# DoHoonKim8/stark-verifier

Hardware: AMD Instinct MI355X
Metric: recursive plonky2 proofs/sec (Semaphore d=20) (higher is better)
Workload: dtype u64 (Goldilocks field, integer); 1 GPU; recursive: per unit one Semaphore signal (group 2^20, n=2^13, blowup 8, 28 FRI queries, 16 PoW bits, zk) + the recursive proof verifying it (n=2^14, same FRI parameters); 128 units per GPU per step, 10 prover contexts per GPU; all_gather of (nullifier|topic) + Poseidon aggregation root per step; parallelism=independent proofs sharded over ranks, no data-path collective, exchange=none (one rank): gl355_aggregation_root over the local leaves, units_proven_in_process=1674

## Files before the change

stark-verifier_amd/csrc/merkle.hip:

```cpp
#include "gl355_internal.h"
#include "poseidon.cuh"
#include "merkle_common.cuh"

namespace gl355 {


__global__ void __launch_bounds__(256) poseidon_permute_kernel(uint64_t* states, uint64_t count) {
    const uint64_t i = blockIdx.x * (uint64_t)blockDim.x + threadIdx.x;
    if (i >= count) return;
    uint64_t s[12];
#pragma unroll
    for (int k = 0; k < 12; k++) s[k] = states[i * 12 + k];
    psd_permute(s);
#pragma unroll
    for (int k = 0; k < 12; k++) states[i * 12 + k] = gl_canon(s[k]);
}


#ifndef PSD_LEAF_WAVES
#define PSD_LEAF_WAVES 4
#endif
__global__ void __launch_bounds__(256) __attribute__((amdgpu_waves_per_eu(PSD_LEAF_WAVES))) hash_leaves_kernel(LeafArgs a) {
    const uint64_t i = blockIdx.x * (uint64_t)blockDim.x + threadIdx.x;
    if (i >= a.n_leaves) return;
    uint64_t s[12];
#pragma unroll
    for (int k = 0; k < 12; k++) s[k] = 0;
    const uint32_t len = a.leaf_len;
    uint64_t d[4];
    if (len <= 4 && !a.always_hash) {
        for (uint32_t k = 0; k < 4; k++) {
            uint64_t v = 0;
            if (k < len) v = leaf_elem(a, i, k);
            d[k] = gl_canon(v);
        }
    } else {
        for (uint32_t off = 0; off < len; off += 8) {
            const uint32_t m = min(8u, len - off);
#pragma unroll
            for (uint32_t k = 0; k < 8; k++) {
                if (k < m) s[k] = leaf_elem(a, i, off + k);
            }
            psd_permute(s);
        }
#pragma unroll
        for (int k = 0; k < 4; k++) d[k] = gl_canon(s[k]);
    }
    uint64_t* dst;
    if (a.linear) dst = a.out + i * 4;
    else if (a.sub_bits == 0) dst = a.cap + i * 4;
    else {
        const uint64_t sub_leaves = 1ull << a.sub_bits;
        const uint64_t t = i >> a.sub_bits, k = i & (sub_leaves - 1);
        dst = a.out + (t * 2 * (sub_leaves - 1) + digest_slot(0, k)) * 4;
    }
    *reinterpret_cast<ulonglong2*>(dst) = make_ulonglong2(d[0], d[1]);
    *reinterpret_cast<ulonglong2*>(dst + 2) = make_ulonglong2(d[2], d[3]);
}

__global__ void __launch_bounds__(256) merkle_level_kernel(uint64_t* digests, uint64_t* cap, uint32_t sub_bits,
                                                          uint32_t layer, uint64_t n_nodes ) {
    const uint64_t g = blockIdx.x * (uint64_t)blockDim.x + threadIdx.x;
    if (g >= n_nodes) return;
    const uint64_t sub_leaves = 1ull << sub_bits;
    const uint64_t per = sub_leaves >> layer;
    const uint64_t t = g / per, k = g % per;
    uint64_t* tree = digests + t * 2 * (sub_leaves - 1) * 4;
    const uint64_t child = digest_slot(layer - 1, 2 * k);
    const ulonglong2 l0 = *reinterpret_cast<const ulonglong2*>(tree + child * 4);
    const ulonglong2 l1 = *reinterpret_cast<const ulonglong2*>(tree + child * 4 + 2);
    const ulonglong2 r0 = *reinterpret_cast<const ulonglong2*>(tree + child * 4 + 4);
    const ulonglong2 r1 = *reinterpret_cast<const ulonglong2*>(tree + child * 4 + 6);
    uint64_t s[12] = {l0.x, l0.y, l1.x, l1.y, r0.x, r0.y, r1.x, r1.y, 0, 0, 0, 0};
    psd_permute(s);
    uint64_t* dst = (layer == sub_bits) ? cap + t * 4 : tree + digest_slot(layer, k) * 4;
    *reinterpret_cast<ulonglong2*>(dst) = make_ulonglong2(gl_canon(s[0]), gl_canon(s[1]));
    *reinterpret_cast<ulonglong2*>(dst + 2) = make_ulonglong2(gl_canon(s[2]), gl_canon(s[3]));
}

__device__ __constant__ const uint32_t PSD_CIRC_DEV[12] = {17, 15, 41, 16, 2, 28, 13, 13, 39, 18, 34, 20};

#define GL_WAVE_LDS_SYNC()                                      \
    do {                                                        \
        __builtin_amdgcn_fence(__ATOMIC_SEQ_CST, "wavefront");  \
        __builtin_amdgcn_wave_barrier();                        \
    } while (0)
#ifndef PSD_LANES_FORM
#define PSD_LANES_FORM -1
#endif
template <int FORM>
GL_DEV uint64_t psd_permute_lanes(uint64_t s, int li, uint64_t* ring ) {
    const bool active = li < 12;
    const int me = active ? li : 0;
    s = gl_add_canonical(s, PSD_ALL_RC[me]);
    auto dense_round = [&](int r, bool full) {
        const uint64_t rc_next = PSD_ALL_RC[12 * (r + 1) + me];
        if (full || li == 0) s = psd_sbox(s);
        if (active) { ring[me] = s; ring[me + 12] = s; }
        GL_WAVE_LDS_SYNC();
        uint64_t al = (uint32_t)rc_next, ah = rc_next >> 32;
#pragma unroll
        for (int j = 0; j < 12; j++) {
            const uint64_t x = ring[me + j];
            const uint32_t c = PSD_CIRC_DEV[j] + ((me == 0 && j == 0) ? 8u : 0u);
            al += (uint64_t)(uint32_t)x * c;
            ah += (uint64_t)(uint32_t)(x >> 32) * c;
        }
        GL_WAVE_LDS_SYNC();
        s = psd_recombine(al, ah);
    };
#if !defined(__HIP_DEVICE_COMPILE__) || GL_MUL_VARIANT != 1
#pragma unroll 1
    for (int r = 0; r < 30; r++) dense_round(r, r < 4 || r >= 26);
#else
    if constexpr (FORM == 0) {
#pragma unroll 1
        for (int r = 0; r < 30; r++) dense_round(r, r < 4 || r >= 26);
        return s;
    }
    const uint32_t c_elem0 = PSD_CIRC_DEV[(12 - me) % 12] + (me == 0 ? 8u : 0u);
#pragma unroll 1
    for (int r = 0; r < 4; r++) dense_round(r, true);
#pragma unroll 1
    for (int r = 4; r < 26; r++) {
        const uint64_t rc_next = PSD_ALL_RC[12 * (r + 1) + me];
        if (active) { const uint64_t pub = li == 0 ? 0 : s; ring[me] = pub; ring[me + 12] = pub; }
        GL_WAVE_LDS_SYNC();
        uint64_t xr[12];
#pragma unroll
        for (int j = 0; j < 12; j++) xr[j] = ring[me + j];
        uint64_t al = (uint32_t)rc_next, ah = rc_next >> 32;
        auto term = [&](int j) {
            al += (uint64_t)(uint32_t)xr[j] * PSD_CIRC_DEV[j];
            ah += (uint64_t)(uint32_t)(xr[j] >> 32) * PSD_CIRC_DEV[j];
        };
        const uint64_t x2 = gl_mul_fill(s, s, [&](int k) { term(k); });
        uint64_t p34[2];
        { const uint64_t pa[2] = {s, x2}, pb[2] = {x2, x2}; gl_mul2_fill(pa, pb, p34, [&](int k) { term(5 + k); }); }
        const uint64_t x7 = gl_mul_fill(p34[0], p34[1], [&](int k) { if (k < 2) term(10 + k); else asm volatile("s_nop 1"); });
        const uint32_t x0l = __builtin_amdgcn_update_dpp(0u, (uint32_t)x7, 0x150, 0xf, 0xf, false);
        const uint32_t x0h = __builtin_amdgcn_update_dpp(0u, (uint32_t)(x7 >> 32), 0x150, 0xf, 0xf, false);
        al += (uint64_t)x0l * c_elem0;
        ah += (uint64_t)x0h * c_elem0;
        GL_WAVE_LDS_SYNC();
        s = psd_recombine(al, ah);
    }
#pragma unroll 1
    for (int r = 26; r < 30; r++) dense_round(r, true);
#endif
    return s;
}

template <int FORM>
__global__ void __launch_bounds__(64) merkle_level_lanes_kernel(uint64_t* digests, uint64_t* cap, uint32_t sub_bits,
                                                               uint32_t layer, uint64_t n_nodes) {
    __shared__ uint64_t rings[4][24];
    const int li = threadIdx.x & 15, grp = threadIdx.x >> 4;
    uint64_t g = blockIdx.x * 4ull + grp;
    const bool valid = g < n_nodes;
    if (!valid) g = 0;
    const uint64_t sub_leaves = 1ull << sub_bits;
    const uint64_t per = sub_leaves >> layer;
    const uint64_t t = g / per, k = g % per;
    uint64_t* tree = digests + t * 2 * (sub_leaves - 1) * 4;
    const uint64_t child = digest_slot(layer - 1, 2 * k);
    uint64_t s = (li < 8) ? tree[child * 4 + li] : 0;
    s = psd_permute_lanes<FORM>(s, li, rings[grp]);
    if (valid && li < 4) {
        uint64_t* dst = (layer == sub_bits) ? cap + t * 4 : tree + digest_slot(layer, k) * 4;
        dst[li] = gl_canon(s);
    }
}

#define MERKLE_TOP_LEVELS 8
template <int FORM>
__global__ void __launch_bounds__(1024) merkle_top_kernel(uint64_t* digests, uint64_t* cap, uint32_t sub_bits, uint32_t layer0, uint32_t n_levels) {
    __shared__ uint64_t rings[64][24];
    __shared__ uint64_t lvl[2][(1 << (MERKLE_TOP_LEVELS - 1)) * 4];
    const int li = threadIdx.x & 15, grp = threadIdx.x >> 4;
    const int wave_first_grp = (threadIdx.x >> 6) << 2;
    const uint64_t sub_leaves = 1ull << sub_bits;
    const uint64_t t = blockIdx.x;
    uint64_t* tree = digests + t * 2 * (sub_leaves - 1) * 4;
    int cur = 0;
    for (uint32_t l = 0; l < n_levels; l++) {
        const uint32_t layer = layer0 + l;
        const int cnt = 1 << (n_levels - 1 - l);
        for (int base = 0; base < cnt; base += 64) {
            if (base + wave_first_grp < cnt) {
                const bool valid = base + grp < cnt;
                const int j = valid ? base + grp : 0;
                uint64_t s = 0;
                if (li < 8) s = (l == 0) ? tree[digest_slot(layer - 1, 2 * (uint64_t)j) * 4 + li] : lvl[cur][(2 * j) * 4 + li];
                s = psd_permute_lanes<FORM>(s, li, rings[grp]);
                if (valid && li < 4) {
                    const uint64_t v = gl_canon(s);
                    lvl[cur ^ 1][j * 4 + li] = v;
                    uint64_t* dst = (layer == sub_bits) ? cap + t * 4 : tree + digest_slot(layer, (uint64_t)j) * 4;
                    dst[li] = v;
                }
            }
        }
        __syncthreads();
        cur ^= 1;
    }
}

__global__ void __launch_bounds__(256) two_to_one_kernel(const uint64_t* l, const uint64_t* r, uint64_t n, uint64_t* out) {
    const uint64_t i = blockIdx.x * (uint64_t)blockDim.x + threadIdx.x;
    if (i >= n) return;
    uint64_t s[12] = {l[4 * i], l[4 * i + 1], l[4 * i + 2], l[4 * i + 3],
                      r[4 * i], r[4 * i + 1], r[4 * i + 2], r[4 * i + 3], 0, 0, 0, 0};
    psd_permute(s);
#pragma unroll
    for (int k = 0; k < 4; k++) out[4 * i + k] = gl_canon(s[k]);
}

__global__ void __launch_bounds__(256) pow_grind_kernel(const uint64_t* state, uint32_t pos, uint32_t bits,
                                                       uint64_t start, unsigned long long* best) {
    const uint64_t w = start + blockIdx.x * (uint64_t)blockDim.x + threadIdx.x;
    if (w > __hip_atomic_load(best, __ATOMIC_RELAXED, __HIP_MEMORY_SCOPE_AGENT)) return;
    uint64_t s[12];
#pragma unroll
    for (int k = 0; k < 12; k++) s[k] = state[k];
#pragma unroll
    for (int k = 0; k < 12; k++) if ((uint32_t)k == pos) s[k] = w;
    psd_permute(s);
    const uint64_t resp = gl_canon(s[7]);
    if (bits == 0 || (resp >> (64 - bits)) == 0) atomicMin(best, (unsigned long long)w);
}

__global__ void open_batch_kernel(const uint64_t* lde, uint64_t stride, uint32_t leaf_len, const uint64_t* digests,
                                  uint32_t log_n, uint32_t cap_height, const uint64_t* idx, uint32_t idx_shift,
                                  uint64_t* leaves_out, uint64_t leaf_out_stride, uint64_t* sib_out, uint64_t sib_out_stride) {
    const uint64_t index = idx[blockIdx.x] >> idx_shift;
    const uint32_t layers = log_n - cap_height;
    for (uint32_t c = threadIdx.x; c < leaf_len; c += blockDim.x)
        leaves_out[(uint64_t)blockIdx.x * leaf_out_stride + c] = stride ? lde[(uint64_t)c * stride + index] : lde[index * leaf_len + c];
    const uint64_t sub_leaves = 1ull << layers;
    const uint64_t* tree = digests + (index >> layers) * 2 * (sub_leaves - 1) * 4;
    const uint64_t k0 = index & (sub_leaves - 1);
    for (uint32_t e = threadIdx.x; e < layers * 4; e += blockDim.x) {
        const uint32_t layer = e >> 2;
        const uint64_t k = (k0 >> layer) ^ 1;
        sib_out[(uint64_t)blockIdx.x * sib_out_stride + layer * 4 + (e & 3)] = tree[digest_slot(layer, k) * 4 + (e & 3)];
    }
}

int32_t open_batch_dev(Ctx* ctx, const uint64_t* lde, uint64_t stride, uint32_t leaf_len, const uint64_t* digests,
                       uint32_t log_n, uint32_t cap_height, const uint64_t* idx_dev, uint32_t n_idx, uint64_t* leaves_out,
                       uint64_t* sib_out) {
    if (n_idx == 0) return GL355_OK;
    ProfScope ps(ctx, "open_batch", (uint64_t)n_idx * (leaf_len * 16 + (log_n - cap_height) * 64));
    hipLaunchKernelGGL(open_batch_kernel, dim3(n_idx), dim3(64), 0, ctx->stream, lde, stride, leaf_len, digests, log_n,
                       cap_height, idx_dev, 0u, leaves_out, (uint64_t)leaf_len, sib_out, (uint64_t)(log_n - cap_height) * 4);
    GL355_HIP(ctx, hipGetLastError());
    return GL355_OK;
}
int32_t open_batch_ex_dev(Ctx* ctx, const uint64_t* leaves, uint64_t stride, uint32_t leaf_len, const uint64_t* digests,
                          uint32_t log_n, uint32_t cap_height, const uint64_t* idx_dev, uint32_t idx_shift, uint32_t n_idx,
                          uint64_t* leaves_out, uint64_t leaf_out_stride, uint64_t* sib_out, uint64_t sib_out_stride) {
    if (n_idx == 0) return GL355_OK;
    ProfScope ps(ctx, "open_batch", (uint64_t)n_idx * (leaf_len * 16 + (log_n - cap_height) * 64));
    hipLaunchKernelGGL(open_batch_kernel, dim3(n_idx), dim3(64), 0, ctx->stream, leaves, stride, leaf_len, digests, log_n,
                       cap_height, idx_dev, idx_shift, leaves_out, leaf_out_stride, sib_out, sib_out_stride);
    GL355_HIP(ctx, hipGetLastError());
    return GL355_OK;
}

int32_t poseidon_permute_dev(Ctx* ctx, uint64_t* states, uint64_t count) {
    if (count == 0) return GL355_OK;
    hipLaunchKernelGGL(poseidon_permute_kernel, dim3((uint32_t)((count + 255) / 256)), dim3(256), 0, ctx->stream, states, count);
    GL355_HIP(ctx, hipGetLastError());
    return GL355_OK;
}

static int32_t launch_leaves(Ctx* ctx, const LeafArgs& a) {
    if (a.n_leaves == 0) return GL355_OK;
    hipLaunchKernelGGL(hash_leaves_kernel, dim3((uint32_t)((a.n_leaves + 255) / 256)), dim3(256), 0, ctx->stream, a);
    GL355_HIP(ctx, hipGetLastError());
    return GL355_OK;
}

int32_t hash_leaves_dev(Ctx* ctx, const uint64_t* leaves, uint64_t n_leaves, uint32_t leaf_len, bool col_major,
                        uint64_t col_stride, uint64_t* digests) {
    LeafArgs a;
    memset(&a, 0, sizeof a);
    a.leaves = leaves; a.n_leaves = n_leaves; a.leaf_len = leaf_len; a.col_major = col_major;
    a.stride = col_major ? col_stride : leaf_len;
    a.out = digests; a.linear = 1;
    return launch_leaves(ctx, a);
}

int32_t hash_no_pad_dev(Ctx* ctx, const uint64_t* inputs, uint64_t n, uint32_t len, uint64_t* digests) {
    LeafArgs a;
    memset(&a, 0, sizeof a);
    a.leaves = inputs; a.n_leaves = n; a.leaf_len = len; a.col_major = 0; a.stride = len;
    a.out = digests; a.linear = 1; a.always_hash = 1;
    return launch_leaves(ctx, a);
}

int32_t two_to_one_dev(Ctx* ctx, const uint64_t* l, const uint64_t* r, uint64_t n, uint64_t* out) {
    if (n == 0) return GL355_OK;
    hipLaunchKernelGGL(two_to_one_kernel, dim3((uint32_t)((n + 255) / 256)), dim3(256), 0, ctx->stream, l, r, n, out);
    GL355_HIP(ctx, hipGetLastError());
    return GL355_OK;
}

int32_t merkle_build_dev(Ctx* ctx, const uint64_t* leaves, uint64_t n_leaves, uint32_t leaf_len, bool col_major,
                         uint64_t col_stride, uint32_t cap_height, uint64_t* digests, uint64_t* cap) {
// ... 77 lines not shown
```

stark-verifier_amd/csrc/poseidon.cuh:

```cuda
#pragma once
#include "gl_field.cuh"

#define PSD_TABLE_QUAL __device__ __constant__ const
#include "poseidon_tables.h"

namespace gl355 {

#ifndef PSD_SBOX_INTERLEAVE
#define PSD_SBOX_INTERLEAVE 1
#endif
#ifndef PSD_SBOX_WIDTH
#define PSD_SBOX_WIDTH 4
#endif
GL_DEV uint64_t psd_sbox(uint64_t x) {
#if PSD_SBOX_INTERLEAVE && defined(__HIP_DEVICE_COMPILE__) && GL_MUL_VARIANT == 1
    const uint64_t x2 = gl_sqr(x);
    const uint64_t a[2] = {x, x2}, b[2] = {x2, x2};
    uint64_t r[2];
    gl_mul_multi<2>(a, b, r);
    return gl_mul(r[0], r[1]);
#else
    uint64_t x2 = gl_sqr(x), x4 = gl_sqr(x2), x3 = gl_mul(x, x2);
    return gl_mul(x3, x4);
#endif
}
GL_DEV void psd_sbox2(uint64_t& x, uint64_t& y) {
#if PSD_SBOX_INTERLEAVE && defined(__HIP_DEVICE_COMPILE__) && GL_MUL_VARIANT == 1
    uint64_t sq[2];
    { const uint64_t a[2] = {x, y}; gl_mul_multi<2>(a, a, sq); }
    uint64_t r[4];
    { const uint64_t a[4] = {x, sq[0], y, sq[1]}, b[4] = {sq[0], sq[0], sq[1], sq[1]}; gl_mul_multi<4>(a, b, r); }
    { const uint64_t a[2] = {r[0], r[2]}, b[2] = {r[1], r[3]}; uint64_t o[2]; gl_mul_multi<2>(a, b, o); x = o[0]; y = o[1]; }
#else
    x = psd_sbox(x); y = psd_sbox(y);
#endif
}

GL_DEV uint64_t psd_recombine(uint64_t al, uint64_t ah) {
#if GL_MUL_VARIANT == 1 && defined(__HIP_DEVICE_COMPILE__)
    uint32_t t1 = (uint32_t)(al >> 32), top;
    asm("v_add_co_u32_e32 %0, vcc, %0, %2\n\t" GL_HAZARD_NOP "v_addc_co_u32_e32 %1, vcc, 0, %3, vcc"
        : "+v"(t1), "=v"(top) : "v"((uint32_t)ah), "v"((uint32_t)(ah >> 32)) : "vcc");
    return gl_dev_add_mul_eps(((uint64_t)t1 << 32) | (uint32_t)al, top);
#else
    const uint64_t mid = ah << 32;
    const uint32_t top = (uint32_t)(ah >> 32);
    const uint64_t r0 = al + mid;
    const uint64_t carry = r0 < mid ? 1u : 0u;
    const uint64_t t = (uint64_t)(top + carry) * GL_EPS;
    uint64_t r1 = r0 + t;
    if (r1 < t) r1 += GL_EPS;
    return r1;
#endif
}

GL_DEV void psd_sbox4(uint64_t& x0, uint64_t& x1, uint64_t& x2, uint64_t& x3) {
#if PSD_SBOX_INTERLEAVE && defined(__HIP_DEVICE_COMPILE__) && GL_MUL_VARIANT == 1
    const uint64_t a[4] = {x0, x1, x2, x3};
    uint64_t sq[4], c3[4], c4[4], o[4];
    gl_mul_multi<4>(a, a, sq);
    gl_mul_multi<4>(a, sq, c3);
    gl_mul_multi<4>(sq, sq, c4);
    gl_mul_multi<4>(c3, c4, o);
    x0 = o[0]; x1 = o[1]; x2 = o[2]; x3 = o[3];
#else
    x0 = psd_sbox(x0); x1 = psd_sbox(x1); x2 = psd_sbox(x2); x3 = psd_sbox(x3);
#endif
}
template <int N>
GL_DEV void psd_recombine_multi(const uint64_t (&al)[N], const uint64_t (&ah)[N], uint64_t (&out)[N]) {
#if GL_MUL_VARIANT == 1 && defined(__HIP_DEVICE_COMPILE__)
    static_assert(N >= 3, "three or more: no wait states of their own");
    uint32_t t1[N], top[N], m[N];
    uint64_t c[N], r[N];
#pragma unroll
    for (int j = 0; j < N; j++) {
        asm("v_add_co_u32_e64 %0, %1, %2, %3" : "=v"(t1[j]), "=s"(c[j]) : "v"((uint32_t)(al[j] >> 32)), "v"((uint32_t)ah[j]));
        __builtin_amdgcn_sched_barrier(0);
    }
#pragma unroll
    for (int j = 0; j < N; j++) {
        asm("v_addc_co_u32_e64 %0, %1, 0, %2, %1" : "=v"(top[j]), "+s"(c[j]) : "v"((uint32_t)(ah[j] >> 32)));
        __builtin_amdgcn_sched_barrier(0);
    }
#pragma unroll
    for (int j = 0; j < N; j++) {
        const uint64_t x = ((uint64_t)t1[j] << 32) | (uint32_t)al[j];
        asm("v_mad_u64_u32 %0, %1, %2, -1, %3" : "=v"(r[j]), "=s"(c[j]) : "v"(top[j]), "v"(x));
        __builtin_amdgcn_sched_barrier(0);
    }
#pragma unroll
    for (int j = 0; j < N; j++) {
        asm("v_cndmask_b32_e64 %0, 0, -1, %1" : "=v"(m[j]) : "s"(c[j]));
        __builtin_amdgcn_sched_barrier(0);
    }
#pragma unroll
    for (int j = 0; j < N; j++) out[j] = r[j] + (uint64_t)m[j];
#else
#pragma unroll
    for (int j = 0; j < N; j++) out[j] = psd_recombine(al[j], ah[j]);
#endif
}

#define PSD_MDS_CHAIN(C0)                                                                                  \
    "v_mad_u64_u32 %0, %1, %2, " #C0 ", %14\n\tv_mad_u64_u32 %0, %1, %3, 15, %0\n\tv_mad_u64_u32 %0, %1, %4, 41, %0\n\t" \
    "v_mad_u64_u32 %0, %1, %5, 16, %0\n\tv_mad_u64_u32 %0, %1, %6, 2, %0\n\tv_mad_u64_u32 %0, %1, %7, 28, %0\n\t"      \
    "v_mad_u64_u32 %0, %1, %8, 13, %0\n\tv_mad_u64_u32 %0, %1, %9, 13, %0\n\tv_mad_u64_u32 %0, %1, %10, 39, %0\n\t"    \
    "v_mad_u64_u32 %0, %1, %11, 18, %0\n\tv_mad_u64_u32 %0, %1, %12, 34, %0\n\tv_mad_u64_u32 %0, %1, %13, 20, %0"
template <int R>
GL_DEV uint64_t psd_mds_chain(const uint32_t (&x)[12], uint64_t addend) {
    uint64_t acc, unused;
#define PSD_X(i) "v"(x[((i) + R) % 12])
    if constexpr (R == 0)
        asm(PSD_MDS_CHAIN(25) : "=&v"(acc), "=&s"(unused) : PSD_X(0), PSD_X(1), PSD_X(2), PSD_X(3), PSD_X(4), PSD_X(5), PSD_X(6),
            PSD_X(7), PSD_X(8), PSD_X(9), PSD_X(10), PSD_X(11), "s"(addend));
    else
        asm(PSD_MDS_CHAIN(17) : "=&v"(acc), "=&s"(unused) : PSD_X(0), PSD_X(1), PSD_X(2), PSD_X(3), PSD_X(4), PSD_X(5), PSD_X(6),
            PSD_X(7), PSD_X(8), PSD_X(9), PSD_X(10), PSD_X(11), "s"(addend));
#undef PSD_X
    return acc;
}
template <int R>
GL_DEV void psd_mds_rows(uint64_t (&s)[12], const uint32_t (&lo)[12], const uint32_t (&hi)[12], const uint64_t* rc) {
    if constexpr (R < 12) {
#if PSD_SBOX_INTERLEAVE
        const uint64_t c0 = rc[R], c1 = rc[R + 1], c2 = rc[R + 2], c3 = rc[R + 3];
        const uint64_t al[4] = {psd_mds_chain<R>(lo, (uint32_t)c0), psd_mds_chain<R + 1>(lo, (uint32_t)c1), psd_mds_chain<R + 2>(lo, (uint32_t)c2),
                                psd_mds_chain<R + 3>(lo, (uint32_t)c3)};
        const uint64_t ah[4] = {psd_mds_chain<R>(hi, c0 >> 32), psd_mds_chain<R + 1>(hi, c1 >> 32), psd_mds_chain<R + 2>(hi, c2 >> 32),
                                psd_mds_chain<R + 3>(hi, c3 >> 32)};
        uint64_t o[4];
        __builtin_amdgcn_sched_barrier(0);
        psd_recombine_multi<4>(al, ah, o);
        s[R] = o[0]; s[R + 1] = o[1]; s[R + 2] = o[2]; s[R + 3] = o[3];
        psd_mds_rows<R + 4>(s, lo, hi, rc);
#else
        const uint64_t c = rc[R];
        s[R] = psd_recombine(psd_mds_chain<R>(lo, (uint32_t)c), psd_mds_chain<R>(hi, c >> 32));
        psd_mds_rows<R + 1>(s, lo, hi, rc);
#endif
    }
}
GL_DEV void psd_mds(uint64_t (&s)[12], const uint64_t* rc) {
    uint32_t lo[12], hi[12];
#pragma unroll
    for (int i = 0; i < 12; i++) { lo[i] = (uint32_t)s[i]; hi[i] = (uint32_t)(s[i] >> 32); }
    psd_mds_rows<0>(s, lo, hi, rc);
}


#undef PSD_TABLE_QUAL
#define PSD_TABLE_QUAL __device__ __constant__
#include "poseidon_ktables.h"

GL_DEV void psd_split(uint64_t x, uint32_t (&l)[3]) {
    const uint32_t lo = (uint32_t)x, hi = (uint32_t)(x >> 32);
    l[0] = lo & 0x3FFFFFu;
    l[1] = __builtin_amdgcn_alignbit(hi, lo, 22) & 0x3FFFFFu;
    l[2] = hi >> 12;
}
typedef const __attribute__((address_space(4))) uint64_t* psd_ktab;
GL_DEV void psd_mac(uint64_t& lo, uint64_t& hi, const uint32_t (&l)[3], const uint64_t (&c)[3]) {
    const uint64_t c0 = c[0], c1 = c[1], c2 = c[2];
#if defined(__HIP_DEVICE_COMPILE__)
    uint64_t unused;
    asm("v_mad_u64_u32 %0, %2, %3, %9, %0\n\tv_mad_u64_u32 %1, %2, %4, %9, %1\n\t"
        "v_mad_u64_u32 %0, %2, %5, %10, %0\n\tv_mad_u64_u32 %1, %2, %6, %10, %1\n\t"
        "v_mad_u64_u32 %0, %2, %7, %11, %0\n\tv_mad_u64_u32 %1, %2, %8, %11, %1"
        : "+v"(lo), "+v"(hi), "=&s"(unused)
        : "s"((uint32_t)c0), "s"((uint32_t)(c0 >> 32)), "s"((uint32_t)c1), "s"((uint32_t)(c1 >> 32)), "s"((uint32_t)c2), "s"((uint32_t)(c2 >> 32)),
          "v"(l[0]), "v"(l[1]), "v"(l[2]));
#else
    lo += (uint64_t)l[0] * (uint32_t)c0 + (uint64_t)l[1] * (uint32_t)c1 + (uint64_t)l[2] * (uint32_t)c2;
    hi += (uint64_t)l[0] * (uint32_t)(c0 >> 32) + (uint64_t)l[1] * (uint32_t)(c1 >> 32) + (uint64_t)l[2] * (uint32_t)(c2 >> 32);
#endif
}
GL_DEV void psd_mac_first(uint64_t& lo, uint64_t& hi, const uint32_t (&l)[3], const uint64_t (&c)[3], const uint64_t (&add)[2]) {
    const uint64_t c0 = c[0], c1 = c[1], c2 = c[2];
#if defined(__HIP_DEVICE_COMPILE__)
    uint64_t unused;
    asm("v_mov_b64 %0, %12\n\tv_mov_b64 %1, %13\n\t"
        "v_mad_u64_u32 %0, %2, %3, %9, %0\n\tv_mad_u64_u32 %1, %2, %4, %9, %1\n\t"
        "v_mad_u64_u32 %0, %2, %5, %10, %0\n\tv_mad_u64_u32 %1, %2, %6, %10, %1\n\t"
        "v_mad_u64_u32 %0, %2, %7, %11, %0\n\tv_mad_u64_u32 %1, %2, %8, %11, %1"
        : "=&v"(lo), "=&v"(hi), "=&s"(unused)
        : "s"((uint32_t)c0), "s"((uint32_t)(c0 >> 32)), "s"((uint32_t)c1), "s"((uint32_t)(c1 >> 32)), "s"((uint32_t)c2), "s"((uint32_t)(c2 >> 32)),
          "v"(l[0]), "v"(l[1]), "v"(l[2]), "s"(add[0]), "s"(add[1]));
#else
    lo = add[0]; hi = add[1];
    psd_mac(lo, hi, l, c);
#endif
}
#ifndef PSD_K_GROUP
#define PSD_K_GROUP 5
#endif
struct PsdK {
    uint64_t w[PSD_K_GROUP][3];
    uint64_t a[2];
};
template <int N, bool WITH_ADD>
GL_DEV void psd_kload(PsdK& k, psd_ktab c, psd_ktab add) {
#pragma unroll
    for (int i = 0; i < N; i++)
#pragma unroll
        for (int j = 0; j < 3; j++) k.w[i][j] = c[3 * i + j];
    if constexpr (WITH_ADD) { k.a[0] = add[0]; k.a[1] = add[1]; }
}
template <int NX, bool HAS_NEXT, int XCAP>
GL_DEV void psd_dot(const uint32_t (&ul)[11][3], const uint32_t (&xl)[XCAP][3], psd_ktab c, PsdK& k, psd_ktab add_next, uint64_t& lo, uint64_t& hi) {
    constexpr int G = PSD_K_GROUP, NT = 11 + NX, NG = (NT + G - 1) / G;
    PsdK cur = k;
#pragma unroll
    for (int g = 0; g < NG; g++) {
        const int n = NT - g * G < G ? NT - g * G : G;
        PsdK nxt;
#pragma unroll
        for (int i = 0; i < G; i++) {
            const int t = g * G + i;
            if (t == 0) psd_mac_first(lo, hi, ul[0], cur.w[0], cur.a);
            else if (i < n) {
                if (t < 11) psd_mac(lo, hi, ul[t], cur.w[i]);
                else psd_mac(lo, hi, xl[t - 11], cur.w[i]);
            }
            if (i == 0) {
                __builtin_amdgcn_sched_barrier(0);
                if (g + 1 < NG) {
                    if (NT - (g + 1) * G >= G) psd_kload<G, false>(nxt, c + 3 * (g + 1) * G, add_next);
                    else psd_kload<(NT % G ? NT % G : G), false>(nxt, c + 3 * (g + 1) * G, add_next);
                } else if constexpr (HAS_NEXT) {
                    psd_kload<G, true>(nxt, c + 3 * NT, add_next);
                }
                __builtin_amdgcn_sched_barrier(0);
            }
        }
        __builtin_amdgcn_sched_barrier(0);
        if (g + 1 < NG || HAS_NEXT) cur = nxt;
    }
    if constexpr (HAS_NEXT) k = cur;
}
template <int J>
GL_DEV void psd_block_lane0(const uint32_t (&ul)[11][3], uint32_t (&xl)[PSD_K_BLOCK][3], psd_ktab mac, psd_ktab add, PsdK& k) {
    if constexpr (J < PSD_K_BLOCK) {
        uint64_t lo, hi;
        psd_dot<J, true>(ul, xl, mac + 3 * (11 * (J - 1) + (J - 1) * J / 2), k, add + 2 * J, lo, hi);
        psd_split(psd_sbox(psd_recombine(lo, hi)), xl[J]);
        __builtin_amdgcn_sched_barrier(0);
        psd_block_lane0<J + 1>(ul, xl, mac, add, k);
    }
}
template <int R>
GL_DEV void psd_block_out(uint64_t (&s)[12], const uint32_t (&ul)[11][3], const uint32_t (&xl)[PSD_K_BLOCK][3], psd_ktab mac, psd_ktab add, PsdK& k) {
    constexpr int B = PSD_K_BLOCK;
    if constexpr (R < 12) {
        uint64_t lo, hi;
        psd_dot<B, (R < 11)>(ul, xl, mac + 3 * (11 * (B - 1) + (B - 1) * B / 2 + (11 + B) * R), k, add + 2 * (B + R), lo, hi);
        s[R] = psd_recombine(lo, hi);
        __builtin_amdgcn_sched_barrier(0);
        psd_block_out<R + 1>(s, ul, xl, mac, add, k);
    }
}
GL_DEV void psd_partial_rounds_block(uint64_t (&s)[12]) {
    constexpr int B = PSD_K_BLOCK;
#pragma unroll 1
    for (int blk = 0; blk < 22 / B; blk++) {
        psd_ktab add = (psd_ktab)PSD_K_ADD + blk * 2 * (B - 1 + 12);
        psd_ktab mac = (psd_ktab)PSD_K_MAC;
        asm volatile("" : "+s"(mac));
        PsdK k;
        psd_kload<PSD_K_GROUP, true>(k, mac, add);
        __builtin_amdgcn_sched_barrier(0);
        uint32_t ul[11][3], xl[B][3];
#pragma unroll
        for (int i = 0; i < 11; i++) psd_split(s[i + 1], ul[i]);
        psd_split(psd_sbox(s[0]), xl[0]);
        __builtin_amdgcn_sched_barrier(0);
        psd_block_lane0<1>(ul, xl, mac, add, k);
        psd_block_out<0>(s, ul, xl, mac, add, k);
    }
}

#ifndef PSD_PARTIAL_FORM
#define PSD_PARTIAL_FORM 1
#endif
#ifndef PSD_ROUNDS_PER_ITER
#define PSD_ROUNDS_PER_ITER 2
#endif
template <bool FULL>
GL_DEV void psd_dense_rounds(uint64_t (&s)[12], int r0, int r1) {
#pragma unroll 1
    for (int r = r0; r < r1; r += PSD_ROUNDS_PER_ITER) {
#pragma unroll
        for (int h = 0; h < PSD_ROUNDS_PER_ITER; h++) {
            if (FULL) {
#pragma unroll
#if PSD_SBOX_WIDTH == 4
                for (int i = 0; i < 12; i += 4) psd_sbox4(s[i], s[i + 1], s[i + 2], s[i + 3]);
#else
                for (int i = 0; i < 12; i += 2) psd_sbox2(s[i], s[i + 1]);
#endif
            } else {
                s[0] = psd_sbox(s[0]);
            }
            psd_mds(s, &PSD_ALL_RC[12 * (r + h + 1)]);
        }
    }
}
GL_DEV void psd_permute(uint64_t (&s)[12]) {
#pragma unroll
    for (int i = 0; i < 12; i++) s[i] = gl_add_canonical(s[i], PSD_ALL_RC[i]);
    psd_dense_rounds<true>(s, 0, 4);
#if PSD_PARTIAL_FORM == 1
    psd_partial_rounds_block(s);
#else
    psd_dense_rounds<false>(s, 4, 26);
#endif
    psd_dense_rounds<true>(s, 26, 30);
}

struct PsdSponge {
    uint64_t s[12];
    GL_DEV void init() {
#pragma unroll
        for (int i = 0; i < 12; i++) s[i] = 0;
    }
};

}
```

stark-verifier_amd/csrc/prover_batch.hip:

```cpp
#include "gl355_internal.h"
#include "blinding.cuh"
#include "poseidon.cuh"

using namespace gl355;

namespace gl355 {

constexpr uint32_t MAXB = GL355_MAX_UNITS;

struct BOracle {
    Ctx* ctx = nullptr;
    uint32_t B = 0, log_n = 0, rate_bits = 0, batch = 0, leaf_len = 0, cap_height = 0;
    uint64_t* base = nullptr;
    uint64_t *coeffs = nullptr, *lde = nullptr, *salt = nullptr, *digests = nullptr, *cap = nullptr;
    uint64_t n_dig = 0;
    ~BOracle() { if (base && ctx) ctx->release(base); }
    int32_t alloc(Ctx* c, uint32_t b, uint32_t lg, uint32_t rb, uint32_t bat, bool salted, uint32_t cap_h) {
        ctx = c; B = b; log_n = lg; rate_bits = rb; batch = bat; leaf_len = bat + (salted ? GL355_SALT_SIZE : 0); cap_height = cap_h;
        const uint64_t n = 1ull << lg, N = n << rb, n_cap = 1ull << cap_h;
        n_dig = 2 * (N - n_cap);
        const uint64_t total = (uint64_t)B * ((uint64_t)bat * n + (uint64_t)leaf_len * N + n_dig * 4 + n_cap * 4);
        void* p = nullptr;
        GL355_TRY(c->alloc(total * 8, &p));
        base = reinterpret_cast<uint64_t*>(p);
// ... 254 lines not shown
        if (other < DEEP_BLK) add = gl2_mul(gl2_make(sh[2 * other], sh[2 * other + 1]), gl2_make(z_pow2[2 * s], z_pow2[2 * s + 1]));
        __syncthreads();
        c = gl2_add(c, add);
        sh[2 * tid] = c.c0; sh[2 * tid + 1] = c.c1;
        __syncthreads();
    }
    uint64_t* v = a.v + (uint64_t)u * a.n * 2;
    if (k < a.n) { v[2 * k] = c.c0; v[2 * k + 1] = c.c1; }
    if (tid == 0) { uint64_t* t = a.totals + ((uint64_t)u * a.n_blocks + blockIdx.x) * 2; t[0] = c.c0; t[1] = c.c1; }
}
__global__ void deep_carry_units_kernel(DeepArgs a) {
    const uint32_t u = blockIdx.x;
    if (threadIdx.x != 0) return;
    const uint64_t* tab = deep_tab_u(a, u);
    const uint64_t* z_pows = tab + 2 * ((uint64_t)(a.n_alpha + 1) + (uint64_t)a.point * (8 + DEEP_BLK + 1) + 8);
    const gl2 zb = gl2_make(z_pows[2 * DEEP_BLK], z_pows[2 * DEEP_BLK + 1]);
    const uint64_t* totals = a.totals + (uint64_t)u * a.n_blocks * 2;
    uint64_t* carry = a.carry + (uint64_t)u * a.n_blocks * 2;
    gl2 c = gl2_make(0, 0);
    for (uint64_t blk = a.n_blocks; blk-- > 0;) {
        carry[2 * blk] = c.c0; carry[2 * blk + 1] = c.c1;
        c = gl2_add(gl2_make(totals[2 * blk], totals[2 * blk + 1]), gl2_mul(zb, c));
    }
}
__global__ void __launch_bounds__(DEEP_BLK) deep_finish_units_kernel(DeepArgs a) {
    const uint64_t k = blockIdx.x * (uint64_t)DEEP_BLK + threadIdx.x;
    if (k >= a.n) return;
    const uint32_t u = blockIdx.y;
    const uint64_t* tab = deep_tab_u(a, u);
    const uint64_t* z_pows = tab + 2 * ((uint64_t)(a.n_alpha + 1) + (uint64_t)a.point * (8 + DEEP_BLK + 1) + 8);
    const uint64_t* v = a.v + (uint64_t)u * a.n * 2;
    const uint64_t* carry = a.carry + (uint64_t)u * a.n_blocks * 2;
    gl2 q = gl2_make(0, 0);
    const uint64_t j = k + 1;
    if (j < a.n) {
        const uint64_t blk = j / DEEP_BLK, off = j % DEEP_BLK;
        const gl2 cr = gl2_make(carry[2 * blk], carry[2 * blk + 1]);
        const uint64_t e = DEEP_BLK - off;
        q = gl2_add(gl2_make(v[2 * j], v[2 * j + 1]), gl2_mul(gl2_make(z_pows[2 * e], z_pows[2 * e + 1]), cr));
    }
    uint64_t* acc0 = a.acc + (uint64_t)u * 2 * a.n;
    uint64_t* acc1 = acc0 + a.n;
    const gl2 shift = gl2_make(tab[2 * a.n_polys], tab[2 * a.n_polys + 1]);
    const gl2 r = gl2_canon(gl2_add(gl2_mul(gl2_make(acc0[k], acc1[k]), shift), q));
    acc0[k] = r.c0; acc1[k] = r.c1;
}

__global__ void fri_leaves_units_kernel(const uint64_t* cols , uint64_t len, uint64_t* leaves ) {
    const uint64_t i = blockIdx.x * (uint64_t)blockDim.x + threadIdx.x;
    if (i >= len / 2) return;
    const uint32_t u = blockIdx.y;
    const uint64_t* c0 = cols + (uint64_t)u * 2 * len;
    const uint64_t* c1 = c0 + len;
    const ulonglong2 a = *reinterpret_cast<const ulonglong2*>(c0 + 2 * i);
    const ulonglong2 b = *reinterpret_cast<const ulonglong2*>(c1 + 2 * i);
    uint64_t* dst = leaves + ((uint64_t)u * (len / 2) + i) * 4;
    *reinterpret_cast<ulonglong2*>(dst) = make_ulonglong2(a.x, b.x);
    *reinterpret_cast<ulonglong2*>(dst + 2) = make_ulonglong2(a.y, b.y);
}
__global__ void fri_fold_units_kernel(const uint64_t* cols , uint64_t len, UnitVals beta, uint64_t* out ) {
    const uint64_t k = blockIdx.x * (uint64_t)blockDim.x + threadIdx.x;
    const uint64_t half = len / 2;
    if (k >= half) return;
    const uint32_t u = blockIdx.y;
    const uint64_t* c0 = cols + (uint64_t)u * 2 * len;
    const uint64_t* c1 = c0 + len;
    const ulonglong2 a = *reinterpret_cast<const ulonglong2*>(c0 + 2 * k);
    const ulonglong2 b = *reinterpret_cast<const ulonglong2*>(c1 + 2 * k);
    const gl2 r = gl2_canon(gl2_add(gl2_make(a.x, b.x), gl2_mul(gl2_make(a.y, b.y), gl2_make(beta.v[u * 4], beta.v[u * 4 + 1]))));
    uint64_t* o0 = out + (uint64_t)u * 2 * half;
    o0[k] = r.c0; o0[half + k] = r.c1;
}
struct PowArgs { uint64_t state[MAXB * 12]; uint32_t pos[MAXB]; uint32_t todo[MAXB]; uint32_t bits; uint64_t start; unsigned long long* best; };
__global__ void __launch_bounds__(256) pow_grind_units_kernel(PowArgs a) {
    const uint32_t u = blockIdx.y;
    if (!a.todo[u]) return;
    const uint64_t w = a.start + blockIdx.x * (uint64_t)blockDim.x + threadIdx.x;
    if (w > __hip_atomic_load(a.best + u, __ATOMIC_RELAXED, __HIP_MEMORY_SCOPE_AGENT)) return;
    uint64_t s[12];
#pragma unroll
    for (int k = 0; k < 12; k++) s[k] = a.state[u * 12 + k];
#pragma unroll
    for (int k = 0; k < 12; k++) if ((uint32_t)k == a.pos[u]) s[k] = w;
    psd_permute(s);
    const uint64_t resp = gl_canon(s[7]);
    if (a.bits == 0 || (resp >> (64 - a.bits)) == 0) atomicMin(a.best + u, (unsigned long long)w);
}

struct OpenArgs { OView o; uint64_t N; uint32_t lde_bits, cap_height, n_idx; const uint64_t* idx ; uint64_t* leaves; uint64_t* sibs; };
__global__ void open_units_kernel(OpenArgs a) {
    const uint32_t q = blockIdx.x, u = blockIdx.y;
    const uint64_t index = a.idx[(uint64_t)u * a.n_idx + q];
    const uint32_t layers = a.lde_bits - a.cap_height;
    const uint64_t* lde = a.o.lde + (uint64_t)u * a.o.lde_us;
    const uint64_t* salt = a.o.salt ? a.o.salt + (uint64_t)u * a.o.salt_us : nullptr;
    uint64_t* lo = a.leaves + ((uint64_t)u * a.n_idx + q) * a.o.leaf_len;
    for (uint32_t c = threadIdx.x; c < a.o.leaf_len; c += blockDim.x)
        lo[c] = c < a.o.batch ? lde[(uint64_t)c * a.N + index] : salt[(uint64_t)(c - a.o.batch) * a.N + index];
    const uint64_t sub_leaves = 1ull << layers;
    const uint64_t* tree = a.o.digests + (uint64_t)u * a.o.dig_us + (index >> layers) * 2 * (sub_leaves - 1) * 4;
    const uint64_t k0 = index & (sub_leaves - 1);
    uint64_t* so = a.sibs + ((uint64_t)u * a.n_idx + q) * layers * 4;
    for (uint32_t e = threadIdx.x; e < layers * 4; e += blockDim.x) {
        const uint32_t layer = e >> 2;
        const uint64_t k = (k0 >> layer) ^ 1;
        so[e] = tree[digest_slot(layer, k) * 4 + (e & 3)];
    }
}
struct OpenFriArgs {
    const uint64_t* trees; uint64_t leaf_off[32], dig_off[32];
    uint64_t sib_off[32], sib_total;
    uint32_t lde_bits, cap_height, n_idx, n_layers;
    const uint64_t* idx; uint64_t* evals ; uint64_t* sibs ;
};
__global__ void open_fri_units_kernel(OpenFriArgs a) {
    const uint32_t q = blockIdx.x, u = blockIdx.y, l = blockIdx.z;
    const uint64_t index = a.idx[(uint64_t)u * a.n_idx + q] >> (l + 1);
    const uint32_t log_nl = a.lde_bits - 1 - l, layers = log_nl - a.cap_height;
    const uint64_t nl = 1ull << log_nl, n_cap = 1ull << a.cap_height;
    const uint64_t* leaves = a.trees + a.leaf_off[l] + (uint64_t)u * nl * 4;
    const uint64_t* digs = a.trees + a.dig_off[l] + (uint64_t)u * 2 * (nl - n_cap) * 4;
    uint64_t* ev = a.evals + (((uint64_t)u * a.n_idx + q) * a.n_layers + l) * 4;
    if (threadIdx.x < 4) ev[threadIdx.x] = leaves[index * 4 + threadIdx.x];
    const uint64_t sub_leaves = 1ull << layers;
    const uint64_t* tree = digs + (index >> layers) * 2 * (sub_leaves - 1) * 4;
    const uint64_t k0 = index & (sub_leaves - 1);
    uint64_t* so = a.sibs + ((uint64_t)u * a.n_idx + q) * a.sib_total + a.sib_off[l];
    for (uint32_t e = threadIdx.x; e < layers * 4; e += blockDim.x) {
        const uint32_t layer = e >> 2;
        const uint64_t k = (k0 >> layer) ^ 1;
        so[e] = tree[digest_slot(layer, k) * 4 + (e & 3)];
    }
}

#define LAUNCH_CHECK(ctx) GL355_HIP(ctx, hipGetLastError())

static int32_t commit_units(Ctx* ctx, int32_t hasher, BOracle& o, bool is_coeffs, bool canonical, const UnitKeys* keys, uint32_t stream_id) {
    const uint64_t n = 1ull << o.log_n, N = n << o.rate_bits;
    const uint32_t cols = o.B * o.batch, lde_bits = o.log_n + o.rate_bits;
    if (!is_coeffs) GL355_TRY(ntt_dev(ctx, o.coeffs, o.log_n, cols, n, true, 0));
    else if (!canonical) GL355_TRY(canon_dev(ctx, o.coeffs, (uint64_t)cols * n));
    GL355_TRY(lde_dev(ctx, o.coeffs, n, o.log_n, o.rate_bits, GL355_COSET_SHIFT, cols, o.lde, N, true));
    if (o.salt) {
        const uint64_t cnt = (uint64_t)GL355_SALT_SIZE * N;
        ProfScope ps(ctx, "salt", cnt * 8 * o.B);
        hipLaunchKernelGGL(salt_units_kernel, dim3((uint32_t)((cnt / 4 + 255) / 256), o.B), dim3(256), 0, ctx->stream, o.salt, lde_bits, *keys, stream_id);
        LAUNCH_CHECK(ctx);
    }
    LeafArgs a;
    memset(&a, 0, sizeof a);
    a.leaves = o.lde; a.n_leaves = (uint64_t)o.B * N; a.leaf_len = o.leaf_len; a.col_major = 1; a.stride = N;
    a.unit_log = lde_bits; a.n_main = o.batch; a.unit_stride = (uint64_t)o.batch * N; a.salt = o.salt; a.salt_unit_stride = (uint64_t)GL355_SALT_SIZE * N;
    return merkle_build_args_any(ctx, hasher, a, lde_bits - o.cap_height, o.digests, o.cap);
}

int32_t prove_units(Ctx* ctx, const gl355_prover_data* pd, uint32_t B, const uint64_t* d_wires_dense, const uint32_t* row_idx,
                    const uint64_t* rows_host, uint32_t n_rows, uint32_t blind_start, uint32_t n_blind, uint32_t z_start, uint32_t n_z_pairs,
                    const ProveUnit* io) {
    if (!pd || !pd->circuit || !pd->constants_sigmas || !pd->sigmas || !pd->k_is || !io || B == 0 || B > MAXB)
        return ctx->fail(GL355_E_INVALID_ARG, "prove: null argument or more than GL355_MAX_UNITS units");
    struct CpuScope {
        Ctx* c; uint64_t t0;
        explicit CpuScope(Ctx* cx) : c(cx), t0(cx->prof_on ? thread_cpu_ns() : 0) {}
        ~CpuScope() { if (c->prof_on) { c->prove_cpu_ns += thread_cpu_ns() - t0; c->prove_calls++; } }
    } cpu_scope(ctx);
    const gl355_circuit& c = *pd->circuit;
    const uint32_t nch = c.num_challenges, qdf = c.max_degree, npp = c.num_partial_products, routed = c.num_routed_wires, nw = c.num_wires;
// ... 364 lines not shown
```

Before: 314.8 recursive proofs/s.

## Specialise Poseidon permutation for zero capacity and partially consumed outputs

Adds a specialised Poseidon permutation that skips work the call site does not need. When the capacity lanes start at zero, the first round skips their constant additions and S-boxes and uses a precomputed folded MDS constant table. On the last round it computes only the output row groups the caller reads: the digest for Merkle and compression, the PoW lane, or the next absorb's surviving lanes for leaf hashing. This cuts arithmetic in the hash-heavy kernels, at the cost of correctness depending on the new fold constants and the per-site group masks being exactly right.

```diff
diff --git a/stark-verifier_amd/csrc/merkle.hip b/stark-verifier_amd/csrc/merkle.hip
--- a/stark-verifier_amd/csrc/merkle.hip
+++ b/stark-verifier_amd/csrc/merkle.hip
@@ -41,7 +41,8 @@
             for (uint32_t k = 0; k < 8; k++) {
                 if (k < m) s[k] = leaf_elem(a, i, off + k);
             }
-            psd_permute(s);
+            const uint32_t rest = len - off - m;
+            psd_permute_spec(s, off == 0, rest == 0 ? 1u : rest >= 8 ? 4u : rest >= 4 ? 6u : 7u);
         }
 #pragma unroll
         for (int k = 0; k < 4; k++) d[k] = gl_canon(s[k]);
@@ -72,7 +73,7 @@
     const ulonglong2 r0 = *reinterpret_cast<const ulonglong2*>(tree + child * 4 + 4);
     const ulonglong2 r1 = *reinterpret_cast<const ulonglong2*>(tree + child * 4 + 6);
     uint64_t s[12] = {l0.x, l0.y, l1.x, l1.y, r0.x, r0.y, r1.x, r1.y, 0, 0, 0, 0};
-    psd_permute(s);
+    psd_permute_spec(s, true, 1u);
     uint64_t* dst = (layer == sub_bits) ? cap + t * 4 : tree + digest_slot(layer, k) * 4;
     *reinterpret_cast<ulonglong2*>(dst) = make_ulonglong2(gl_canon(s[0]), gl_canon(s[1]));
     *reinterpret_cast<ulonglong2*>(dst + 2) = make_ulonglong2(gl_canon(s[2]), gl_canon(s[3]));
@@ -211,7 +212,7 @@
     if (i >= n) return;
     uint64_t s[12] = {l[4 * i], l[4 * i + 1], l[4 * i + 2], l[4 * i + 3],
                       r[4 * i], r[4 * i + 1], r[4 * i + 2], r[4 * i + 3], 0, 0, 0, 0};
-    psd_permute(s);
+    psd_permute_spec(s, true, 1u);
 #pragma unroll
     for (int k = 0; k < 4; k++) out[4 * i + k] = gl_canon(s[k]);
 }
@@ -225,7 +226,7 @@
     for (int k = 0; k < 12; k++) s[k] = state[k];
 #pragma unroll
     for (int k = 0; k < 12; k++) if ((uint32_t)k == pos) s[k] = w;
-    psd_permute(s);
+    psd_permute_spec(s, false, 2u);
     const uint64_t resp = gl_canon(s[7]);
     if (bits == 0 || (resp >> (64 - bits)) == 0) atomicMin(best, (unsigned long long)w);
 }
diff --git a/stark-verifier_amd/csrc/poseidon.cuh b/stark-verifier_amd/csrc/poseidon.cuh
--- a/stark-verifier_amd/csrc/poseidon.cuh
+++ b/stark-verifier_amd/csrc/poseidon.cuh
@@ -102,6 +102,7 @@
 #endif
 }
 
+constexpr int PSD_CIRC_COEF[12] = {17, 15, 41, 16, 2, 28, 13, 13, 39, 18, 34, 20};
 #define PSD_MDS_CHAIN(C0)                                                                                  \
     "v_mad_u64_u32 %0, %1, %2, " #C0 ", %14\n\tv_mad_u64_u32 %0, %1, %3, 15, %0\n\tv_mad_u64_u32 %0, %1, %4, 41, %0\n\t" \
     "v_mad_u64_u32 %0, %1, %5, 16, %0\n\tv_mad_u64_u32 %0, %1, %6, 2, %0\n\tv_mad_u64_u32 %0, %1, %7, 28, %0\n\t"      \
@@ -120,38 +121,75 @@
 #undef PSD_X
     return acc;
 }
+template <int R, int J>
+GL_DEV void psd_fold_step(uint64_t& acc, const uint32_t (&x)[12], uint64_t addend) {
+    constexpr int C = PSD_CIRC_COEF[(J - R + 12) % 12] + ((R == 0 && J == 0) ? 8 : 0);
+    uint64_t unused;
+    if constexpr (J == 0)
+        asm("v_mad_u64_u32 %0, %1, %2, %3, %4" : "=&v"(acc), "=&s"(unused) : "v"(x[0]), "I"(C), "s"(addend));
+    else
+        asm("v_mad_u64_u32 %0, %1, %2, %3, %0" : "+v"(acc), "=&s"(unused) : "v"(x[J]), "I"(C));
+    if constexpr (J < 7) psd_fold_step<R, J + 1>(acc, x, addend);
+}
 template <int R>
-GL_DEV void psd_mds_rows(uint64_t (&s)[12], const uint32_t (&lo)[12], const uint32_t (&hi)[12], const uint64_t* rc) {
+GL_DEV uint64_t psd_fold_chain(const uint32_t (&x)[12], uint64_t addend) {
+    uint64_t acc;
+#if defined(__HIP_DEVICE_COMPILE__)
+    psd_fold_step<R, 0>(acc, x, addend);
+#else
+    acc = addend;
+    for (int j = 0; j < 8; j++) acc += (uint64_t)x[j] * (uint64_t)(PSD_CIRC_COEF[(j - R + 12) % 12] + ((R == 0 && j == 0) ? 8 : 0));
+#endif
+    return acc;
+}
+
+template <int R, bool FOLD>
+GL_DEV void psd_mds_rows(uint64_t (&s)[12], const uint32_t (&lo)[12], const uint32_t (&hi)[12], const uint64_t* rc, uint32_t groups) {
     if constexpr (R < 12) {
 #if PSD_SBOX_INTERLEAVE
-        const uint64_t c0 = rc[R], c1 = rc[R + 1], c2 = rc[R + 2], c3 = rc[R + 3];
-        const uint64_t al[4] = {psd_mds_chain<R>(lo, (uint32_t)c0), psd_mds_chain<R + 1>(lo, (uint32_t)c1), psd_mds_chain<R + 2>(lo, (uint32_t)c2),
-                                psd_mds_chain<R + 3>(lo, (uint32_t)c3)};
-        const uint64_t ah[4] = {psd_mds_chain<R>(hi, c0 >> 32), psd_mds_chain<R + 1>(hi, c1 >> 32), psd_mds_chain<R + 2>(hi, c2 >> 32),
-                                psd_mds_chain<R + 3>(hi, c3 >> 32)};
-        uint64_t o[4];
-        __builtin_amdgcn_sched_barrier(0);
-        psd_recombine_multi<4>(al, ah, o);
-        s[R] = o[0]; s[R + 1] = o[1]; s[R + 2] = o[2]; s[R + 3] = o[3];
-        psd_mds_rows<R + 4>(s, lo, hi, rc);
-#else
-        const uint64_t c = rc[R];
-        s[R] = psd_recombine(psd_mds_chain<R>(lo, (uint32_t)c), psd_mds_chain<R>(hi, c >> 32));
-        psd_mds_rows<R + 1>(s, lo, hi, rc);
-#endif
-    }
-}
-GL_DEV void psd_mds(uint64_t (&s)[12], const uint64_t* rc) {
+        if (groups & (1u << (R / 4))) {
+            const uint64_t c0 = rc[R], c1 = rc[R + 1], c2 = rc[R + 2], c3 = rc[R + 3];
+            uint64_t al[4], ah[4];
+            if constexpr (FOLD) {
+                al[0] = psd_fold_chain<R>(lo, (uint32_t)c0); al[1] = psd_fold_chain<R + 1>(lo, (uint32_t)c1);
+                al[2] = psd_fold_chain<R + 2>(lo, (uint32_t)c2); al[3] = psd_fold_chain<R + 3>(lo, (uint32_t)c3);
+                ah[0] = psd_fold_chain<R>(hi, c0 >> 32); ah[1] = psd_fold_chain<R + 1>(hi, c1 >> 32);
+                ah[2] = psd_fold_chain<R + 2>(hi, c2 >> 32); ah[3] = psd_fold_chain<R + 3>(hi, c3 >> 32);
+            } else {
+                al[0] = psd_mds_chain<R>(lo, (uint32_t)c0); al[1] = psd_mds_chain<R + 1>(lo, (uint32_t)c1);
+                al[2] = psd_mds_chain<R + 2>(lo, (uint32_t)c2); al[3] = psd_mds_chain<R + 3>(lo, (uint32_t)c3);
+                ah[0] = psd_mds_chain<R>(hi, c0 >> 32); ah[1] = psd_mds_chain<R + 1>(hi, c1 >> 32);
+                ah[2] = psd_mds_chain<R + 2>(hi, c2 >> 32); ah[3] = psd_mds_chain<R + 3>(hi, c3 >> 32);
+            }
+            uint64_t o[4];
+            __builtin_amdgcn_sched_barrier(0);
+            psd_recombine_multi<4>(al, ah, o);
+            s[R] = o[0]; s[R + 1] = o[1]; s[R + 2] = o[2]; s[R + 3] = o[3];
+        }
+        psd_mds_rows<R + 4, FOLD>(s, lo, hi, rc, groups);
+#else
+        if (groups & (1u << (R / 4))) {
+            const uint64_t c = rc[R];
+            if constexpr (FOLD) s[R] = psd_recombine(psd_fold_chain<R>(lo, (uint32_t)c), psd_fold_chain<R>(hi, c >> 32));
+            else s[R] = psd_recombine(psd_mds_chain<R>(lo, (uint32_t)c), psd_mds_chain<R>(hi, c >> 32));
+        }
+        psd_mds_rows<R + 1, FOLD>(s, lo, hi, rc, groups);
+#endif
+    }
+}
+template <bool FOLD = false>
+GL_DEV void psd_mds(uint64_t (&s)[12], const uint64_t* rc, uint32_t groups = 7u) {
     uint32_t lo[12], hi[12];
 #pragma unroll
     for (int i = 0; i < 12; i++) { lo[i] = (uint32_t)s[i]; hi[i] = (uint32_t)(s[i] >> 32); }
-    psd_mds_rows<0>(s, lo, hi, rc);
+    psd_mds_rows<0, FOLD>(s, lo, hi, rc, groups);
 }
 
 
 #undef PSD_TABLE_QUAL
 #define PSD_TABLE_QUAL __device__ __constant__
 #include "poseidon_ktables.h"
+#include "poseidon_ftables.h"
 
 GL_DEV void psd_split(uint64_t x, uint32_t (&l)[3]) {
     const uint32_t lo = (uint32_t)x, hi = (uint32_t)(x >> 32);
@@ -286,36 +324,43 @@
 #define PSD_ROUNDS_PER_ITER 2
 #endif
 template <bool FULL>
-GL_DEV void psd_dense_rounds(uint64_t (&s)[12], int r0, int r1) {
+GL_DEV void psd_dense_rounds(uint64_t (&s)[12], int r0, int r1, bool zcap = false, uint32_t groups = 7u) {
 #pragma unroll 1
     for (int r = r0; r < r1; r += PSD_ROUNDS_PER_ITER) {
 #pragma unroll
         for (int h = 0; h < PSD_ROUNDS_PER_ITER; h++) {
+            const bool fold = FULL && zcap && r + h == 0;
             if (FULL) {
 #pragma unroll
 #if PSD_SBOX_WIDTH == 4
-                for (int i = 0; i < 12; i += 4) psd_sbox4(s[i], s[i + 1], s[i + 2], s[i + 3]);
-#else
-                for (int i = 0; i < 12; i += 2) psd_sbox2(s[i], s[i + 1]);
+                for (int i = 0; i < 12; i += 4) if (i < 8 || !fold) psd_sbox4(s[i], s[i + 1], s[i + 2], s[i + 3]);
+#else
+                for (int i = 0; i < 12; i += 2) if (i < 8 || !fold) psd_sbox2(s[i], s[i + 1]);
 #endif
             } else {
                 s[0] = psd_sbox(s[0]);
             }
-            psd_mds(s, &PSD_ALL_RC[12 * (r + h + 1)]);
+            if (fold) psd_mds<true>(s, (const uint64_t*)PSD_K_FOLD);
+            else psd_mds(s, &PSD_ALL_RC[12 * (r + h + 1)], r + h == 29 ? groups : 7u);
         }
     }
 }
-GL_DEV void psd_permute(uint64_t (&s)[12]) {
-#pragma unroll
-    for (int i = 0; i < 12; i++) s[i] = gl_add_canonical(s[i], PSD_ALL_RC[i]);
-    psd_dense_rounds<true>(s, 0, 4);
+#ifndef PSD_SPECIALISE
+#define PSD_SPECIALISE 1
+#endif
+GL_DEV void psd_permute_spec(uint64_t (&s)[12], bool zcap, uint32_t groups) {
+    if (!PSD_SPECIALISE) { zcap = false; groups = 7u; }
+#pragma unroll
+    for (int i = 0; i < 12; i++) if (i < 8 || !zcap) s[i] = gl_add_canonical(s[i], PSD_ALL_RC[i]);
+    psd_dense_rounds<true>(s, 0, 4, zcap);
 #if PSD_PARTIAL_FORM == 1
     psd_partial_rounds_block(s);
 #else
     psd_dense_rounds<false>(s, 4, 26);
 #endif
-    psd_dense_rounds<true>(s, 26, 30);
-}
+    psd_dense_rounds<true>(s, 26, 30, false, groups);
+}
+GL_DEV void psd_permute(uint64_t (&s)[12]) { psd_permute_spec(s, false, 7u); }
 
 struct PsdSponge {
     uint64_t s[12];
diff --git a/stark-verifier_amd/csrc/poseidon_ftables.h b/stark-verifier_amd/csrc/poseidon_ftables.h
--- /dev/null
+++ b/stark-verifier_amd/csrc/poseidon_ftables.h
@@ -0,0 +1,11 @@
+#pragma once
+#include <stdint.h>
+#ifndef PSD_TABLE_QUAL
+#define PSD_TABLE_QUAL static const
+#endif
+PSD_TABLE_QUAL uint64_t PSD_K_FOLD[12] = {
+  UINT64_C(0x62cfea8e55341db8), UINT64_C(0x53ae0d422f8cc6ef), UINT64_C(0xac29b888aeef84d6),
+  UINT64_C(0x90cc491f71b5fd4e), UINT64_C(0x638cd97d1f14244c), UINT64_C(0xf3fc76291302124d),
+  UINT64_C(0xc57293658eb53e57), UINT64_C(0x60bea017e5f8e6a2), UINT64_C(0x54c44c3971082de9),
+  UINT64_C(0xb7d39352c39511f2), UINT64_C(0xb39c19ddc44cc469), UINT64_C(0x301a0d485cf527f6),
+};
diff --git a/stark-verifier_amd/csrc/prover_batch.hip b/stark-verifier_amd/csrc/prover_batch.hip
--- a/stark-verifier_amd/csrc/prover_batch.hip
+++ b/stark-verifier_amd/csrc/prover_batch.hip
@@ -360,7 +360,7 @@
     for (int k = 0; k < 12; k++) s[k] = a.state[u * 12 + k];
 #pragma unroll
     for (int k = 0; k < 12; k++) if ((uint32_t)k == a.pos[u]) s[k] = w;
-    psd_permute(s);
+    psd_permute_spec(s, false, 2u);
     const uint64_t resp = gl_canon(s[7]);
     if (a.bits == 0 || (resp >> (64 - a.bits)) == 0) atomicMin(a.best + u, (unsigned long long)w);
 }
```

Measured after the change: 317.3 recursive proofs/s (median of 6 runs). Within noise of the previous version (+0.8%).
